# Axionis47/GAT-Recommendation

Hardware: AMD Instinct MI355X
Metric: training sessions/sec + Recall@10 parity, 82k-node graph, 1/2/4/8 MI355X (higher is better)
Workload: dtype fp32

## Files before the change

### gat-recommendation_amd/csrc/gtr_common.cuh

```cuda
#pragma once

#include <hip/hip_runtime.h>
#include <stdint.h>
#include <stdlib.h>

#include "../../include/gtr.h"

#define GTR_BLOCK 256
#define GTR_WAVES (GTR_BLOCK / 64)

typedef float f32x4 __attribute__((ext_vector_type(4)));

namespace gtr {

void set_error(const char* fmt, ...);

struct Buf {
  __amdgpu_buffer_rsrc_t r;
  __device__ __forceinline__ Buf(const void* p, uint64_t bytes)
      : r(__builtin_amdgcn_make_buffer_rsrc(const_cast<void*>(p), (short)0,
                                            (int)(uint32_t)(bytes < 0xFFFFFFFFull ? bytes : 0xFFFFFFFFull),
                                            0x00020000)) {}
  __device__ __forceinline__ float4 ld4(uint32_t off) const {
    return __builtin_bit_cast(float4, __builtin_amdgcn_raw_buffer_load_b128(r, (int)off, 0, 0));
// ... 158 lines not shown
  const int lane = threadIdx.x & 63;
  int lo = 0, hi = B;
  while (hi - lo > 64) {
    const int step = (hi - lo + 63) >> 6;
    const int idx = lo + lane * step;
    const int val = idx < hi ? a[idx] : 0x7FFFFFFF;
    const int c = __popcll(__ballot(val < v));
    const int nlo = c > 0 ? lo + (c - 1) * step + 1 : lo;
    const int nhi = min(hi, lo + c * step);
    lo = nlo;
    hi = nhi;
  }
  const int idx = lo + lane;
  const int val = idx < hi ? a[idx] : 0x7FFFFFFF;
  return lo + __popcll(__ballot(val < v));
}

__device__ __forceinline__ void group_rows(const int32_t* node_ptr, int B, int R, int g, int& r0, int& r1) {
  const int s0 = wave_lower_bound(node_ptr, B, g * R);
  const int s1 = wave_lower_bound(node_ptr, B, (g + 1) * R);
  r0 = node_ptr[s0];
  r1 = node_ptr[s1];
}

__device__ __forceinline__ int role_block(int M, int pack) {
  const int b = blockIdx.x;
  if (!pack) return b;
  if ((b & 7) == 0 && (b >> 3) < M) return b >> 3;
  return M + b - min(M, (b + 7) >> 3);
}

__device__ __forceinline__ bool arrive_last(uint32_t* cnt, uint32_t total, int* s_flag) {
  asm volatile("s_waitcnt vmcnt(0)" ::: "memory");
  __syncthreads();
  if (threadIdx.x == 0) {
    __builtin_amdgcn_fence(__ATOMIC_RELEASE, "agent");
    asm volatile("s_waitcnt vmcnt(0)" ::: "memory");
    uint32_t prev = __hip_atomic_fetch_add(cnt, 1u, __ATOMIC_RELAXED, __HIP_MEMORY_SCOPE_AGENT);
    *s_flag = (prev == total - 1) ? 1 : 0;
  }
  __syncthreads();
  if (*s_flag == 0) return false;
  if (threadIdx.x == 0) {
    __builtin_amdgcn_fence(__ATOMIC_ACQUIRE, "agent");
    asm volatile("s_waitcnt vmcnt(0)" ::: "memory");
  }
  __syncthreads();
  return true;
}

__device__ __forceinline__ void st_wt(float* p, float v) {
  __hip_atomic_store((__attribute__((address_space(1))) uint32_t*)(p), __float_as_uint(v),
                     __ATOMIC_RELAXED, __HIP_MEMORY_SCOPE_AGENT);
}

__device__ __forceinline__ bool arrive_last_wt(uint32_t* cnt, uint32_t total, int* s_flag) {
  asm volatile("s_waitcnt vmcnt(0)" ::: "memory");
  __syncthreads();
  if (threadIdx.x == 0) {
    uint32_t prev = __hip_atomic_fetch_add(cnt, 1u, __ATOMIC_RELAXED, __HIP_MEMORY_SCOPE_AGENT);
    *s_flag = (prev == total - 1) ? 1 : 0;
  }
  __syncthreads();
  if (*s_flag == 0) return false;
  if (threadIdx.x == 0) {
    __builtin_amdgcn_fence(__ATOMIC_ACQUIRE, "agent");
    asm volatile("s_waitcnt vmcnt(0)" ::: "memory");
  }
  __syncthreads();
  return true;
}

__device__ __forceinline__ void reset_counter(uint32_t* cnt) {
  __hip_atomic_store(cnt, 0u, __ATOMIC_RELAXED, __HIP_MEMORY_SCOPE_AGENT);
}

template <int BLK>
__device__ __forceinline__ void block_sum_rows(const float* p, int G, int W, size_t stride, float* out,
                                               float* scr, bool wt = false) {
  const int tid = threadIdx.x;
  if (W >= BLK) {
    for (int j = tid; j < W; j += BLK) {
      float acc = 0.0f;
#pragma unroll 32
      for (int q = 0; q < G; ++q) acc += p[(size_t)q * stride + j];
      if (wt) st_wt(out + j, acc); else out[j] = acc;
    }
    __syncthreads();
    return;
  }
  const int NSL = BLK / W;
  const int j = tid % W, sl = tid / W;
  if (sl < NSL) {
    float acc = 0.0f;
#pragma unroll 32
    for (int q = sl; q < G; q += NSL) acc += p[(size_t)q * stride + j];
    scr[sl * W + j] = acc;
  }
  __syncthreads();
  if (tid < W) {
    float t = 0.0f;
    for (int q = 0; q < NSL; ++q) t += scr[q * W + tid];
    if (wt) st_wt(out + tid, t); else out[tid] = t;
  }
  __syncthreads();
}
// ... 174 lines not shown
```

### gat-recommendation_amd/csrc/gtr_opt.hip

```cpp

#include <hipcub/hipcub.hpp>
#include <rocprim/device/device_radix_sort.hpp>

#include <cstdarg>
#include <cstdio>

#include "gtr_rows.cuh"
#include <string.h>

#include "gtr_wgrad.cuh"

namespace gtr {

static thread_local char g_err[512] = "";

void set_error(const char* fmt, ...) {
  va_list ap;
  va_start(ap, fmt);
  vsnprintf(g_err, sizeof(g_err), fmt, ap);
  va_end(ap);
}

}

// ... 521 lines not shown
      s_st.init(a.opt, t);
      s_t = (int32_t)t;
      s_ready = 1;
    }
    __syncthreads();
  }
  auto wait = [&]() {
    while (__hip_atomic_load(&s_ready, __ATOMIC_ACQUIRE, __HIP_MEMORY_SCOPE_WORKGROUP) == 0)
      __builtin_amdgcn_s_sleep(1);
  };
  const int blk = blockIdx.x;
  if (blk == 0 && tid == 0 && a.tl.rng_inc) *a.tl.rng_inc += 1;
  if (blk < a.nb_rows && a.windowed) {
    wait();
    const AdamStep st = s_st;
    window_rows<D>(blk, a.bt, a.T, a.tl, st, a.tl.lazy_consts ? a.tl.stamp : nullptr, s_t);
    return;
  }
  if (blk < a.nb_rows) {
    rows_body<D>(blk * GTR_BLOCK + tid, a.bt, a.T, a.tl.skeys, a.tl.svals, a.tl.dx0, a.tl.se, a.tl.coef_tgt,
                 a.tl.coef_neg, a.tl.table, a.tl.table_m, a.tl.table_v, nullptr, s_st,
                 a.tl.lazy_consts ? a.tl.stamp : nullptr, s_t, wait);
    return;
  }
  if (blk < a.nb_rows + a.nb_small) {
    const int sb = blk - a.nb_rows;
    small_body((int64_t)sb * GTR_BLOCK + tid, a.segs, a.nseg, a.bt.hdr, a.tl.flat, a.tl.flat_m, a.tl.flat_v, nullptr,
               s_st, wait);
    if (sb == 0 && a.tl.loss_part) {
      float acc = 0.0f;
      for (int q = tid; q < a.tl.loss_nparts; q += GTR_BLOCK)
        acc += a.tl.loss_part[(size_t)q * 2] + a.tl.loss_part[(size_t)q * 2 + 1];
      s_acc[tid] = acc;
      __syncthreads();
      if (tid == 0) {
        float t = 0.0f;
        for (int q = 0; q < GTR_BLOCK; ++q) t += s_acc[q];
        a.tl.loss_out[0] = t;
        if (a.tl.loss_acc) a.tl.loss_acc[0] += (double)t;
      }
    } else if (sb == 0 && a.tl.loss_acc && tid == 0) {
      a.tl.loss_acc[0] += (double)a.tl.loss_out[0];
    }
    return;
  }
  wait();
  const AdamStep st = s_st;
  sweep_body(blk - a.nb_rows - a.nb_small, a.nb_sweep, a.nvec, a.vpr_log2, a.tl.stamp, s_t,
             reinterpret_cast<float4*>(a.tl.table), reinterpret_cast<float4*>(a.tl.table_m),
             reinterpret_cast<float4*>(a.tl.table_v), st, a.vbegin);
}

#define GTR_TAILW_SEGS 16
#define GTR_WT_LIST 4352
struct TailWK {
  gtr_batch bt;
  gtr_tail tl;
  gtr_adam opt;
  int T, nb_rows, nb_wg, nb_small, njobs, D, nseg, P;
  int64_t stride;
  int small_total, pad0;
  uint32_t* cnt;
  gtr_segment segs[GTR_TAILW_SEGS];
  WJob jobs[GTR_MAX_WJOBS];
};

template <int D>
__global__ __launch_bounds__(GTR_BLOCK) void k_step_tail_wgrad(TailWK a) {
  __shared__ AdamStep s_st;
  __shared__ int32_t s_t;
  __shared__ float s_acc[GTR_BLOCK];
  __shared__ uint32_t s_list[GTR_WT_LIST];
  __shared__ int s_n;
  __shared__ int s_flag;
  const int tid = threadIdx.x;
  if (tid == 0) {
    const int64_t t = *a.opt.step_dev + a.opt.step_offset;
    s_st.init(a.opt, t);
    s_t = (int32_t)t;
    s_n = 0;
  }
  __syncthreads();
  const AdamStep st = s_st;
  int blk = blockIdx.x;
  if (blk == 0 && tid == 0 && a.tl.rng_inc) *a.tl.rng_inc += 1;
  if (blk < a.nb_wg) {
    int jid = 0;
    while (jid + 1 < a.njobs && blk >= a.jobs[jid + 1].blk0) ++jid;
    const WJob& J = a.jobs[jid];
    const int local = blk - J.blk0;
    const int tile = local / a.P, p = local - tile * a.P;
    const int N = a.bt.hdr[0];
    const int per = (N + a.P - 1) / a.P;
    const int t0 = p * per, t1 = min(N, t0 + per);
    const int64_t so = (int64_t)p * a.stride;
    auto rec = [&](uint32_t code) { s_list[atomicAdd(&s_n, 1)] = code; };
    auto emit = [&](int which, int64_t idx, float v) {
      if (which == 0) J.outW[so + idx] = v;
      else J.outB[so + idx] = v;
      rec(((uint32_t)which << 30) | (uint32_t)idx);
    };
    auto emit4 = [&](int64_t idx, float4 v) {
      *reinterpret_cast<float4*>(J.outW + so + idx) = v;
      rec((2u << 30) | (uint32_t)idx);
    };
    if (J.mfma == 1) wgrad_tile_mfma<false>(J, tile, t0, t1, emit, emit4);
    else if (J.mfma == 2) wgrad_tile_mfma<true>(J, tile, t0, t1, emit, emit4);
    else wgrad_tile(J, tile, t0, t1, a.D, emit);
    if (!arrive_last(a.cnt + J.tile0 + tile, (uint32_t)a.P, &s_flag)) return;
    const int n = s_n;
    float* P = a.tl.flat;
    float* M = a.tl.flat_m;
    float* V = a.tl.flat_v;
    for (int k = tid; k < n; k += GTR_BLOCK) {
      const uint32_t code = s_list[k];
      const uint32_t kind = code >> 30;
      const int64_t idx = code & 0x3FFFFFFFu;
      const float* src = kind == 1 ? J.outB : J.outW;
      const int64_t f0 = kind == 1 ? J.fB : J.fW;
      const int cnt = kind == 2 ? 4 : 1;
      for (int c = 0; c < cnt; ++c) {
        float g = 0.0f;
        for (int q = 0; q < a.P; ++q) g += src[(int64_t)q * a.stride + idx + c];
        const int64_t e = f0 + idx + c;
        float pv = P[e], mv = M[e], vv = V[e];
        st.apply(pv, mv, vv, g);
        P[e] = pv;
        M[e] = mv;
        V[e] = vv;
      }
    }
    if (tid == 0) reset_counter(a.cnt + J.tile0 + tile);
    return;
  }
  blk -= a.nb_wg;
  if (blk < a.nb_rows) {
    rows_body<D>(blk * GTR_BLOCK + tid, a.bt, a.T, a.tl.skeys, a.tl.svals, a.tl.dx0, a.tl.se, a.tl.coef_tgt,
                 a.tl.coef_neg, a.tl.table, a.tl.table_m, a.tl.table_v, nullptr, st,
                 a.tl.lazy_consts ? a.tl.stamp : nullptr, s_t);
    return;
  }
  blk -= a.nb_rows;
  if (blk < a.nb_small) {
    int64_t i = (int64_t)blk * GTR_BLOCK + tid;
    if (i < a.small_total) {
      int sg = 0;
      while (i >= a.segs[sg].len) { i -= a.segs[sg].len; ++sg; }
      const gtr_segment& S = a.segs[sg];
      float g = 0.0f;
      for (int q = 0; q < S.nparts; ++q) g += S.src[(int64_t)q * S.pstride + i];
      const int64_t e = S.begin + i;
      float pv = a.tl.flat[e], mv = a.tl.flat_m[e], vv = a.tl.flat_v[e];
      st.apply(pv, mv, vv, g);
      a.tl.flat[e] = pv;
      a.tl.flat_m[e] = mv;
      a.tl.flat_v[e] = vv;
    }
    if (blk == 0 && a.tl.loss_part) {
      float acc = 0.0f;
      for (int q = tid; q < a.tl.loss_nparts; q += GTR_BLOCK)
        acc += a.tl.loss_part[(size_t)q * 2] + a.tl.loss_part[(size_t)q * 2 + 1];
      s_acc[tid] = acc;
      __syncthreads();
      if (tid == 0) {
        float t = 0.0f;
        for (int q = 0; q < GTR_BLOCK; ++q) t += s_acc[q];
        a.tl.loss_out[0] = t;
        if (a.tl.loss_acc) a.tl.loss_acc[0] += (double)t;
      }
    } else if (blk == 0 && a.tl.loss_acc && tid == 0) {
      a.tl.loss_acc[0] += (double)a.tl.loss_out[0];
    }
  }
}

template <int D>
__global__ __launch_bounds__(GTR_BLOCK) void k_scatter_rows(gtr_batch bt, int mode, const float* src,
                                                            const float* coef_tgt, const float* coef_neg,
                                                            float* dense) {
  constexpr int VPL = D >= 64 ? D / 64 : 1;
  const int lane = threadIdx.x & 63, wave = threadIdx.x >> 6;
  const int r = blockIdx.x * GTR_WAVES + wave;
  const int d0 = lane * VPL;
  if (d0 >= D) return;
  const int N = bt.hdr[0], B = bt.hdr[1];
  int key;
  const float* s;
  float c;
  if (mode == 0) {
    if (r >= N) return;
    key = bt.node_item[r];
    s = src + (size_t)r * D;
    c = 1.0f;
  } else {
    if (r >= B * (1 + bt.n_neg)) return;
    if (r < B) {
      key = bt.target[r];
      s = src + (size_t)r * D;
      c = coef_tgt[r];
    } else {
      const int q = r - B;
      key = bt.negatives[q];
      s = src + (size_t)(q / bt.n_neg) * D;
      c = coef_neg[q];
    }
// ... 898 lines not shown
#define GTR_TAIL(DD) if (k.windowed) hipLaunchKernelGGL((k_step_tail<DD, false>), dim3(grid), dim3(GTR_BLOCK), 0, s, k); \
  else hipLaunchKernelGGL((k_step_tail<DD, true>), dim3(grid), dim3(GTR_TAIL_BLOCK), 0, s, k)
    case 32: GTR_TAIL(32); break;
    case 64: GTR_TAIL(64); break;
    case 128: GTR_TAIL(128); break;
    default: GTR_TAIL(256); break;
#undef GTR_TAIL
  }
  GTR_HIP_CHECK_LAUNCH();
  return GTR_OK;
}

int gtr_step_tail_wgrad(const gtr_config* cfg, const gtr_batch* bt, const gtr_layer* layers, const float* pe_tab,
                        float* const* layer_slab, float* pe_slab, int n_chunks, int64_t slab_stride,
                        const int64_t* layer_flat, const int64_t* pe_flat, int num_items, const gtr_tail* tail,
                        const gtr_segment* segs, int nseg, const gtr_adam* opt, uint32_t* tile_cnt, int tile_cnt_len,
                        gtr_stream_t stream) {
  if (!cfg || !bt || !layers || !layer_slab || !layer_flat || !tail || !opt || !opt->step_dev || num_items <= 0 ||
      nseg < 0 || nseg > GTR_TAILW_SEGS || (nseg > 0 && !segs) || !dim_ok(cfg->dim) || n_chunks <= 0 ||
      !tile_cnt || 3 * cfg->num_layers + 1 > GTR_MAX_WJOBS) {
    set_error("gtr_step_tail_wgrad: bad arguments");
    return GTR_E_ARG;
  }
  const gtr_tail& t = *tail;
  const int D = cfg->dim;
  const int m_cap = bt->n_cap + bt->b_cap * (1 + bt->n_neg);
  if (m_cap > GTR_BEGIN_MCAP) {
    set_error("gtr_step_tail_wgrad: batch too large (m_cap %d > %d): use gtr_wgrad + gtr_step_tail", m_cap,
              GTR_BEGIN_MCAP);
    return GTR_E_ARG;
  }
  if (!t.lazy_consts && t.sweep_from < num_items) {
    set_error("gtr_step_tail_wgrad: the untouched-row sweep must run in the chain (sweep_from == num_items)");
    return GTR_E_ARG;
  }
  if (!t.skeys || !t.svals || !t.dx0 || !t.se || !t.coef_tgt || !t.coef_neg || !t.table || !t.table_m ||
      !t.table_v || !t.stamp || !t.flat || !t.flat_m || !t.flat_v || (t.loss_part && (!t.loss_out || t.loss_nparts < 0))) {
    set_error("gtr_step_tail_wgrad: missing buffers");
    return GTR_E_ARG;
  }
  TailWK k{};
  k.bt = *bt;
  k.tl = t;
  k.opt = *opt;
  k.T = num_items;
  k.D = D;
  k.P = n_chunks;
  k.stride = slab_stride;
  k.cnt = tile_cnt;
  const char* wm = getenv("GTR_WGRAD");
  bool mfma = (bt->n_cap + n_chunks - 1) / n_chunks >= GTR_WGRAD_MFMA_ROWS;
  if (wm && !strcmp(wm, "mfma")) mfma = true;
  if (wm && !strcmp(wm, "valu")) mfma = false;
  if (slab_stride % 4) mfma = false;
  for (int l = 0; l < cfg->num_layers; ++l)
    if (reinterpret_cast<uintptr_t>(layer_slab[l]) % 16) mfma = false;
  int nj = 0, wblocks = 0;
  const int rc = build_wjobs(cfg, bt, layers, t.dx0, pe_tab, layer_slab, pe_slab, layer_flat, pe_flat, n_chunks, 0,
                             cfg->num_layers, k.jobs, nj, wblocks, mfma);
  if (rc) return rc;
  int tiles = 0;
  for (int i = 0; i < nj; ++i) {
    k.jobs[i].tile0 = tiles;
    tiles += k.jobs[i].nt;
    if (k.jobs[i].fW < 0 && k.jobs[i].fB < 0) { set_error("gtr_step_tail_wgrad: a job without flat offsets"); return GTR_E_ARG; }
  }
  if (tiles > tile_cnt_len) {
    set_error("gtr_step_tail_wgrad: %d tile counters needed, %d given", tiles, tile_cnt_len);
    return GTR_E_ARG;
  }
  k.njobs = nj;
  k.nb_wg = wblocks;
  k.nb_rows = (int)(((int64_t)m_cap * (D / 4) + GTR_BLOCK - 1) / GTR_BLOCK);
  int64_t tot = 0;
  for (int i = 0; i < nseg; ++i) {
    if (segs[i].live_groups) { set_error("gtr_step_tail_wgrad: folded (per row group) weight gradients"); return GTR_E_ARG; }
    k.segs[i] = segs[i];
    tot += segs[i].len;
  }
  k.nseg = nseg;
  k.small_total = (int)tot;
  k.nb_small = (int)((tot + GTR_BLOCK - 1) / GTR_BLOCK);
  if (k.nb_small == 0 && (t.loss_part || t.loss_acc)) k.nb_small = 1;
  const int grid = k.nb_wg + k.nb_rows + k.nb_small;
  hipStream_t s = (hipStream_t)stream;
  switch (D) {
    case 32: hipLaunchKernelGGL(k_step_tail_wgrad<32>, dim3(grid), dim3(GTR_BLOCK), 0, s, k); break;
    case 64: hipLaunchKernelGGL(k_step_tail_wgrad<64>, dim3(grid), dim3(GTR_BLOCK), 0, s, k); break;
    case 128: hipLaunchKernelGGL(k_step_tail_wgrad<128>, dim3(grid), dim3(GTR_BLOCK), 0, s, k); break;
    default: hipLaunchKernelGGL(k_step_tail_wgrad<256>, dim3(grid), dim3(GTR_BLOCK), 0, s, k); break;
  }
  GTR_HIP_CHECK_LAUNCH();
  return GTR_OK;
}

static bool dp_layout_ok(const gtr_dp_layout* l, int dim) {
  return l && l->world >= 1 && l->m_cap > 0 && l->flat_total >= 0 && l->loss_off >= l->flat_total &&
         l->keys_off > l->loss_off && l->rows_off >= l->keys_off + l->m_cap && (l->rows_off & 3) == 0 &&
         l->words >= l->rows_off + (int64_t)l->m_cap * dim && (l->words & 3) == 0;
}

int gtr_dp_pack(const gtr_batch* bt, int num_items, int dim, const gtr_tail* tail, const gtr_segment* segs, int nseg,
                const gtr_dp_layout* lay, float* pack, gtr_stream_t stream) {
  if (!bt || !tail || !pack || !dim_ok(dim) || !dp_layout_ok(lay, dim) || nseg < 0 || nseg > GTR_SMALL_MAX_SEG ||
      lay->m_cap != bt->n_cap + bt->b_cap * (1 + bt->n_neg) || !tail->skeys || !tail->svals || !tail->dx0 ||
      !tail->se || !tail->coef_tgt || !tail->coef_neg || (!tail->loss_part && !tail->loss_out)) {
    set_error("gtr_dp_pack: bad arguments");
    return GTR_E_ARG;
  }
  DpPackK k{};
  k.bt = *bt;
  k.tl = *tail;
  k.lay = *lay;
  k.pack = pack;
  k.T = num_items;
  hipStream_t s = (hipStream_t)stream;
  k.windowed = lay->m_cap > GTR_BEGIN_MCAP ? 1 : 0;
  if (k.windowed) {
    if (!tail->carry) { set_error("gtr_dp_pack: large batch (m_cap > %d) needs the carry scratch", GTR_BEGIN_MCAP); return GTR_E_ARG; }
    const int nwin = (lay->m_cap + TW - 1) / TW;
    k.nb_rows = nwin;
    if (nwin > 1) {
      switch (dim) {
        case 32: hipLaunchKernelGGL(k_tail_carry<32>, dim3(carry_blocks(lay->m_cap)), dim3(GTR_BLOCK), 0, s, *bt, num_items, *tail); break;
        case 64: hipLaunchKernelGGL(k_tail_carry<64>, dim3(carry_blocks(lay->m_cap)), dim3(GTR_BLOCK), 0, s, *bt, num_items, *tail); break;
        case 128: hipLaunchKernelGGL(k_tail_carry<128>, dim3(carry_blocks(lay->m_cap)), dim3(GTR_BLOCK), 0, s, *bt, num_items, *tail); break;
        default: hipLaunchKernelGGL(k_tail_carry<256>, dim3(carry_blocks(lay->m_cap)), dim3(GTR_BLOCK), 0, s, *bt, num_items, *tail); break;
      }
      GTR_HIP_CHECK_LAUNCH();
    }
  } else {
    k.nb_rows = (int)(((int64_t)lay->m_cap * (dim / 4) + GTR_BLOCK - 1) / GTR_BLOCK);
  }
  k.nb_small = (int)((lay->flat_total + GTR_BLOCK - 1) / GTR_BLOCK);
  if (k.nb_small == 0) k.nb_small = 1;
  k.nseg = nseg;
  for (int i = 0; i < nseg; ++i) k.segs[i] = segs[i];
  const int grid = k.nb_rows + k.nb_small;
  switch (dim) {
    case 32: hipLaunchKernelGGL(k_dp_pack<32>, dim3(grid), dim3(GTR_BLOCK), 0, s, k); break;
    case 64: hipLaunchKernelGGL(k_dp_pack<64>, dim3(grid), dim3(GTR_BLOCK), 0, s, k); break;
    case 128: hipLaunchKernelGGL(k_dp_pack<128>, dim3(grid), dim3(GTR_BLOCK), 0, s, k); break;
    default: hipLaunchKernelGGL(k_dp_pack<256>, dim3(grid), dim3(GTR_BLOCK), 0, s, k); break;
// ... 60 lines not shown
```

### gat-recommendation_amd/csrc/gtr_wgrad.cuh

```cuda
#pragma once

#include "gtr_common.cuh"

#include <type_traits>

namespace gtr {

enum { WJ_MM = 0, WJ_GATE = 1, WJ_COLSUM = 2 };

struct WJob {
  int type, M1, M2, lda, ldb, tn, nt, blk0;
  int mfma, wm, wn, fold_bias;
  const float* A;
  const float* B;
  const int32_t* bidx;
  const float* agg;
  const float* s;
  float* outW;
  float* outB;
  int64_t fW, fB;
  int tile0, pad_t;
};

#define GTR_MAX_WJOBS 16

#ifndef GTR_WGRAD_MFMA_ROWS
#define GTR_WGRAD_MFMA_ROWS 128
#endif

struct WgradK {
  const int32_t* hdr;
  int P, njobs, D, pad0;
  int64_t stride;
  WJob jobs[GTR_MAX_WJOBS];
};

template <class Emit>
__device__ __forceinline__ void wgrad_tile(const WJob& J, int tile, int t0, int t1, int D, Emit&& emit) {
  constexpr int TK = 32;
  __shared__ __attribute__((aligned(16))) float As[TK][64];
  __shared__ __attribute__((aligned(16))) float Bs[TK][64];
  const int tid = threadIdx.x;
  if (J.type == WJ_GATE || J.type == WJ_COLSUM) {
    constexpr int PH = GTR_BLOCK / 16;
    __shared__ float4 part[3][PH][16];
    const int c16 = tid & 15, ph = tid >> 4;
    const int col = tile * 64 + c16 * 4;
    const bool gate = J.type == WJ_GATE;
    const int ncol = gate ? D : J.M1;
    float4 g0 = make_float4(0.f, 0.f, 0.f, 0.f), g1 = g0, g2 = g0;
    if (col < ncol) {
      if (gate) {
        const float* ag = J.agg + col;
        const float* sk = J.s + col;
#pragma unroll 4
        for (int t = t0 + ph; t < t1; t += PH) {
          const float u = J.A[t];
          const float4 x = *reinterpret_cast<const float4*>(ag + (size_t)t * D);
          const float4 y = *reinterpret_cast<const float4*>(sk + (size_t)t * J.lda);
          g0.x += u * x.x; g0.y += u * x.y; g0.z += u * x.z; g0.w += u * x.w;
          g1.x += u * y.x; g1.y += u * y.y; g1.z += u * y.z; g1.w += u * y.w;
          g2.x += u * (x.x - y.x); g2.y += u * (x.y - y.y); g2.z += u * (x.z - y.z); g2.w += u * (x.w - y.w);
        }
      } else {
        const float* cp = J.A + col;
#pragma unroll 4
        for (int t = t0 + ph; t < t1; t += PH) {
          const float4 x = *reinterpret_cast<const float4*>(cp + (size_t)t * J.lda);
          g0.x += x.x; g0.y += x.y; g0.z += x.z; g0.w += x.w;
        }
      }
    }
    part[0][ph][c16] = g0;
    if (gate) {
      part[1][ph][c16] = g1;
      part[2][ph][c16] = g2;
    }
    __syncthreads();
    const int nseg = gate ? 3 : 1;
    if (tid < 64 * nseg) {
      const int sg = tid >> 6, cl = tid & 63, cc = cl >> 2, comp = cl & 3;
      const int j = tile * 64 + cl;
      float g = 0.0f;
#pragma unroll
      for (int q = 0; q < PH; ++q) {
        const float4 v = part[sg][q][cc];
        g += comp == 0 ? v.x : comp == 1 ? v.y : comp == 2 ? v.z : v.w;
      }
      if (j < ncol) {
        if (gate) emit(0, sg * D + j, g);
        else emit(1, j, g);
// ... 8 lines not shown
#pragma unroll
  for (int i = 0; i < 4; ++i)
#pragma unroll
    for (int k = 0; k < 4; ++k) acc[i][k] = 0.0f;
  constexpr int NQ = TK * 64 / GTR_BLOCK;
  float av[NQ], bv[NQ];
  auto load = [&](int tb) {
#pragma unroll
    for (int q = 0; q < NQ; ++q) {
      const int idx = tid + q * GTR_BLOCK;
      const int i = idx >> 6, c = idx & 63;
      const int t = tb + i;
      av[q] = 0.0f;
      bv[q] = 0.0f;
      if (t < t1) {
        if (m0 + c < J.M1) av[q] = J.A[(size_t)t * J.lda + m0 + c];
        const int col = n0 + c;
        if (col < J.M2) {
          const float* brow = J.bidx ? J.B + (size_t)J.bidx[t] * J.ldb : J.B + (size_t)t * J.ldb;
          bv[q] = brow[col];
        } else if (col == J.M2) {
          bv[q] = 1.0f;
        }
      }
    }
  };
  if (t0 < t1) load(t0);
  for (int tb = t0; tb < t1; tb += TK) {
#pragma unroll
    for (int q = 0; q < NQ; ++q) {
      const int idx = tid + q * GTR_BLOCK;
      As[idx >> 6][idx & 63] = av[q];
      Bs[idx >> 6][idx & 63] = bv[q];
    }
    __syncthreads();
    if (tb + TK < t1) load(tb + TK);
#pragma unroll 8
    for (int k = 0; k < TK; ++k) {
      const float4 a4 = *reinterpret_cast<const float4*>(&As[k][ty * 4]);
      const float4 b4 = *reinterpret_cast<const float4*>(&Bs[k][tx * 4]);
      const float ar[4] = {a4.x, a4.y, a4.z, a4.w};
      const float br[4] = {b4.x, b4.y, b4.z, b4.w};
#pragma unroll
      for (int i = 0; i < 4; ++i)
#pragma unroll
        for (int q = 0; q < 4; ++q) acc[i][q] += ar[i] * br[q];
    }
    __syncthreads();
  }
#pragma unroll
  for (int i = 0; i < 4; ++i) {
    const int m = m0 + ty * 4 + i;
    if (m >= J.M1) continue;
#pragma unroll
    for (int q = 0; q < 4; ++q) {
      const int nn = n0 + tx * 4 + q;
      if (nn < J.M2) emit(0, (int64_t)m * J.M2 + nn, acc[i][q]);
      else if (nn == J.M2) emit(1, m, acc[i][q]);
    }
  }
}

template <bool NARROW, class Emit, class Emit4>
__device__ __forceinline__ void wgrad_tile_mfma(const WJob& J, int tile, int t0, int t1, Emit&& emit, Emit4&& emit4) {
  constexpr int NT = NARROW ? 2 : 4;
  __shared__ f32x4 red[GTR_WAVES][4][64];
  const int tid = threadIdx.x, lane = tid & 63, wave = tid >> 6;
  const int nw = J.wm * J.wn, kw = GTR_WAVES / nw;
  const int wt = wave % nw, ks = wave / nw;
  const int tm = tile / J.tn, tq = tile - tm * J.tn;
  const int m0 = (tm * J.wm + wt % J.wm) * 64, n0 = (tq * J.wn + wt / J.wm) * 64;
  const int len = t1 - t0, per = (((len + kw - 1) / kw) + 3) & ~3;
  const int r0 = min(t1, t0 + ks * per), r1 = min(t1, r0 + per);
  const int kq = lane >> 4, c4 = (lane & 15) * 4, j16 = lane & 15;
  f32x4 acc[4][NT];
#pragma unroll
  for (int i = 0; i < 4; ++i)
#pragma unroll
    for (int q = 0; q < NT; ++q) acc[i][q] = f32x4{0.f, 0.f, 0.f, 0.f};
  const float* Ap = J.A + m0 + c4;
  const int rlast = max(0, r1 - 1);
  const int jb0 = min(j16, J.M2 - 1), jb1 = min(16 + j16, J.M2 - 1);
  const int32_t* ib = J.bidx ? J.bidx : reinterpret_cast<const int32_t*>(J.A);
  auto idx = [&](int t) -> int {
    const int tc = min(t, rlast);
    const int v = __builtin_nontemporal_load(ib + tc);
    return J.bidx ? v : tc;
  };
  auto ld = [&](int t, int bi, float4& a, float4& b) {
    const int tc = min(t, rlast);
    a = *reinterpret_cast<const float4*>(Ap + (size_t)tc * J.lda);
    if (NARROW) {
      const float* brow = J.B + (size_t)bi * J.ldb;
      b.x = brow[jb0];
      b.y = brow[jb1];
    } else {
      b = *reinterpret_cast<const float4*>(J.B + (size_t)tc * J.ldb + n0 + c4);
    }
  };
  auto fix = [&](int t, float4& a, float4& b) {
    if (t >= r1) {
      a = make_float4(0.f, 0.f, 0.f, 0.f);
      b = a;
    } else if (NARROW) {
      if (j16 >= J.M2) b.x = j16 == J.M2 ? 1.0f : 0.0f;
      if (16 + j16 >= J.M2) b.y = 16 + j16 == J.M2 ? 1.0f : 0.0f;
// ... 52 lines not shown
    stepk(std::integral_constant<int, 2>{}, t + 16);
  }
  if (colsum) {
    cs.x = bfly_add<32>(bfly_add<16>(cs.x)); cs.y = bfly_add<32>(bfly_add<16>(cs.y));
    cs.z = bfly_add<32>(bfly_add<16>(cs.z)); cs.w = bfly_add<32>(bfly_add<16>(cs.w));
  }
  for (int s = 1; s < kw; ++s) {
    if (colsum && ks == s) red[wt][0][lane] = f32x4{cs.x, cs.y, cs.z, cs.w};
    __syncthreads();
    if (colsum && ks == 0) {
      const f32x4 v = red[wt][0][lane];
      cs.x += v[0]; cs.y += v[1]; cs.z += v[2]; cs.w += v[3];
    }
    __syncthreads();
  }
  if (colsum && ks == 0 && kq == 0 && J.fold_bias) {
    emit(1, m0 + c4, cs.x);
    emit(1, m0 + c4 + 1, cs.y);
    emit(1, m0 + c4 + 2, cs.z);
    emit(1, m0 + c4 + 3, cs.w);
  }
  for (int mt = 0; mt < 4; ++mt) {
    for (int s = 1; s < kw; ++s) {
      if (ks == s) {
#pragma unroll
        for (int nt = 0; nt < NT; ++nt) red[wt][nt][lane] = acc[mt][nt];
      }
      __syncthreads();
      if (ks == 0) {
#pragma unroll
        for (int nt = 0; nt < NT; ++nt) acc[mt][nt] += red[wt][nt][lane];
      }
      __syncthreads();
    }
  }
  if (ks != 0) return;
#pragma unroll
  for (int mt = 0; mt < 4; ++mt)
#pragma unroll
    for (int r = 0; r < 4; ++r) {
      const int m = m0 + 16 * kq + 4 * r + mt;
      if (m >= J.M1) continue;
      if (NARROW) {
#pragma unroll
        for (int nt = 0; nt < NT; ++nt) {
          const int nn = 16 * nt + j16;
          if (nn < J.M2) emit(0, (int64_t)m * J.M2 + nn, acc[mt][nt][r]);
          else if (nn == J.M2) emit(1, m, acc[mt][nt][r]);
        }
      } else {
        emit4((int64_t)m * J.M2 + n0 + c4, make_float4(acc[mt][0][r], acc[mt][1][r], acc[mt][2][r], acc[mt][3][r]));
      }
    }
}

inline int build_wjobs(const gtr_config* cfg, const gtr_batch* bt, const gtr_layer* layers, const float* dx0,
                       const float* pe_tab, float* const* layer_slab, float* pe_slab, const int64_t* layer_flat,
                       const int64_t* pe_flat, int n_chunks, int l_begin, int l_end, WJob* jobs, int& nj,
                       int& blocks, bool mfma = false) {
  const int D = cfg->dim;
  nj = 0;
  blocks = 0;
  for (int l = l_begin; l < l_end; ++l) {
    const gtr_layer& L = layers[l];
    float* base = layer_slab ? layer_slab[l] : nullptr;
    const int64_t* fl = layer_flat ? layer_flat + 3 * l : nullptr;
    WJob& w = jobs[nj++];
    w = WJob{};
    w.type = WJ_MM; w.M1 = 4 * D; w.M2 = D; w.lda = 4 * D; w.ldb = D;
    w.tn = (D + 63) / 64; w.nt = ((4 * D + 63) / 64) * w.tn; w.blk0 = blocks;
    if (mfma && D % 64 == 0) {
      w.mfma = 1;
      w.wn = D / 64 >= 2 ? 2 : 1;
      w.wm = GTR_WAVES / w.wn < 4 * D / 64 ? GTR_WAVES / w.wn : 4 * D / 64;
      w.tn = D / (64 * w.wn);
      w.nt = (4 * D / (64 * w.wm)) * w.tn;
      w.fold_bias = 1;
    }
    w.A = L.dqkvs; w.B = L.xin; w.bidx = nullptr;
    w.outW = base; w.outB = base ? base + (size_t)4 * D * D : nullptr;
    w.fW = fl ? fl[0] : -1; w.fB = fl ? fl[1] : -1;
    blocks += w.nt * n_chunks;
    if (D % 64 == 0 && !w.mfma) {
      WJob& c = jobs[nj++];
      c = WJob{};
      c.type = WJ_COLSUM; c.M1 = 4 * D; c.lda = 4 * D; c.tn = 1; c.nt = (4 * D + 63) / 64;
      c.blk0 = blocks; c.A = L.dqkvs; c.outB = base ? base + (size_t)4 * D * D : nullptr;
      c.fW = -1; c.fB = fl ? fl[1] : -1;
      blocks += c.nt * n_chunks;
    }
    WJob& q = jobs[nj++];
    q = WJob{};
    q.type = WJ_GATE; q.M1 = 1; q.M2 = 3 * D; q.lda = 4 * D; q.tn = 1; q.nt = (D + 63) / 64;
    q.blk0 = blocks; q.A = L.du; q.agg = L.agg; q.s = L.qkvs + 3 * D;
    q.outW = base ? base + (size_t)4 * D * D + 4 * D : nullptr;
    q.fW = fl ? fl[2] : -1; q.fB = -1;
    blocks += q.nt * n_chunks;
  }
  if (cfg->pe_k > 0 && (pe_slab || pe_flat) && l_begin == 0) {
    if (!dx0 || (!pe_tab && !bt->node_pe)) { set_error("gtr_wgrad: PE gradient needs dx0 and PE rows"); return GTR_E_ARG; }
    const int K = cfg->pe_k;
    WJob& w = jobs[nj++];
    w = WJob{};
    w.type = WJ_MM; w.M1 = D; w.M2 = K; w.lda = D; w.ldb = K;
    w.tn = (K + 1 + 63) / 64; w.nt = ((D + 63) / 64) * w.tn; w.blk0 = blocks;
    w.A = dx0;
// ... 18 lines not shown
```

### gat-recommendation_amd/etpgt/train/fused.py

```python

from __future__ import annotations

import ctypes as C
import os

import torch

from etpgt.backend import _lib as L
from etpgt.backend.engine import Engine, readout_grid
from etpgt.data.batch import Caps, SessionBatch


class FusedTrainStep:
    def __init__(self, model, lr: float = 1e-3, betas=(0.9, 0.999), eps: float = 1e-8,
                 weight_decay: float = 1e-5, decoupled: bool = True, loss: str = "bpr",
                 temperature: float = 1.0, alpha: float = 0.7, caps: Caps | None = None,
                 use_graph: bool = True, data_parallel: bool | None = None, process_group=None,
                 lazy: bool = False, sync_bn: bool = False, lagged: bool = False, shard_table: bool = False):
        if loss not in ("bpr", "listwise", "dual", "sampled_softmax"):
            raise ValueError(f"Unknown loss type: {loss}")
        if getattr(model, "use_ffn", False):
            if os.environ.get("GTR_TAILW") == "1":
                raise NotImplementedError("the FFN variant (use_ffn=True) has no GTR_TAILW step")
            if sync_bn and not (model.embedding_dim in (64, 128) and getattr(model, "ffn_expansion", 4) == 4):
                raise NotImplementedError("SyncBN with the FFN variant covers dim 64 / 128 at ffn_expansion 4")
        self.model = model
        self.eng: Engine = model.hip_engine()
        self.dev = self.eng.device
        self.loss_kind = L.GTR_LOSS[loss]
        self.temperature = float(temperature)
        self.alpha = float(alpha)
        self.use_graph = use_graph
        from etpgt.train.distributed import world_info

        self.group = process_group
        self.rank, self.world = world_info(process_group)
        self.shard_table = bool(shard_table)
        if self.shard_table and (lazy or lagged):
            raise ValueError("the row-sharded table keeps its own lazy stamps (no lazy/lagged option)")
        self.data_parallel = (self.world > 1) if data_parallel is None else bool(data_parallel)
        self.data_parallel = self.data_parallel or self.shard_table

        self.sync_bn = bool(sync_bn)
        if self.sync_bn and not self.data_parallel:
            raise ValueError("sync_bn needs the data-parallel step")
        self.dp = None
        self.sync_alias = False
        self.graph_b = None
        self._coll_capture_refused = False
        eng = self.eng
        T, D = eng.T, eng.D
        self.adam = L.GtrAdam()
        self.adam.lr, self.adam.beta1, self.adam.beta2 = float(lr), float(betas[0]), float(betas[1])
        self.adam.eps, self.adam.weight_decay, self.adam.decoupled = float(eps), float(weight_decay), int(decoupled)
        self.step_dev = torch.zeros(1, dtype=torch.int64, device=self.dev)
        self.loss_acc = torch.zeros(1, dtype=torch.float64, device=self.dev)
        self.adam.step_dev = self.step_dev.data_ptr()
        self.adam.step_offset = 0
        tab_rows = 1 if self.shard_table else T
        self.m_tab = torch.zeros(tab_rows, D, dtype=torch.float32, device=self.dev)
        self.v_tab = torch.zeros(tab_rows, D, dtype=torch.float32, device=self.dev)
        self.m_flat = torch.zeros_like(eng.flat.flat)
        self.v_flat = torch.zeros_like(eng.flat.flat)
        self.stamp = torch.zeros(tab_rows, dtype=torch.int32, device=self.dev)
        self.lagged = bool(lagged) and not bool(lazy)
        self.lazy = bool(lazy) or self.lagged
# ... 143 lines not shown
        if self.begin_fused:
            wts[0] = 0.0
        self.early_union = (self.data_parallel and chain and not self.sync_bn and not self.lagged
                            and not self.shard_table and os.environ.get("GTR_DP_EARLY", "0") == "1")
        if self.early_union:
            wts = [0.0] * eng.L + wts[eng.L:]
        slots = len(wts)
        if chain and not self.shard_table and not self.split \
                and (not self.data_parallel or self.early_union or self.lagged) \
                and self.ws.g_cap <= 128 and slots <= L.SWEEP_SLOTS:
            sw = L.GtrSweep()
            sw.table = eng.model.item_embedding.weight.data_ptr()
            sw.m, sw.v, sw.stamp = self.m_tab.data_ptr(), self.v_tab.data_ptr(), self.stamp.data_ptr()
            sw.opt = self.adam
            tot, acc = sum(wts), 0.0
            if self.early_union:
                self.keys_all = torch.zeros(self.world, m_cap, dtype=torch.int32, device=self.dev)
            for i in range(L.SWEEP_SLOTS + 1):
                sw.bounds[i] = eng.T if i >= slots else int(eng.T * acc / tot)
                if i < slots:
                    acc += wts[i]
            sw.dim = eng.D
            sw.blocks = int(os.environ.get("GTR_SWEEP_BLOCKS", 0 if eng.D <= 64 else 128))
            sw.lag = 1 if self.lagged else 0
            sw.consts = self.lazy_consts.data_ptr() if self.lagged else None
            self.sweep = sw
            self.cfg.sweep = C.addressof(sw)
            t.sweep_from = eng.T
        t.lazy_consts = self.lazy_consts.data_ptr() if self.lazy else None
        nc = int(L.lib().gtr_tail_carry_floats(m_cap, eng.D))
        self.carry = torch.zeros(max(nc, 4), dtype=torch.float32, device=self.dev) if nc > 0 else None
        t.carry = self.carry.data_ptr() if self.carry is not None else None
        self.cfg.begin, self.cfg.ctr_add, t.rng_inc = None, 0, None
        if self.begin_fused:
            bg = L.GtrBegin()
            bg.skeys, bg.svals, bg.stamp = self.skeys.data_ptr(), self.svals.data_ptr(), self.stamp.data_ptr()
            bg.step_dev, bg.num_items = self.step_dev.data_ptr(), eng.T
            self.begin_st = bg
            self.cfg.begin = C.addressof(bg)
            self.cfg.ctr_add = 1
            t.rng_inc = eng.rng_ctr.data_ptr()
        self.tail = t
        if self.shard_table:
            from etpgt.train.sharded import ShardExchange

            self.dp = None
            self.shard = ShardExchange(self, self.shard_state)
        elif self.data_parallel:
            from etpgt.train.distributed import DpExchange

            self.dp = DpExchange(self, self.group)
        if self.sync_bn:
            self._sync_alloc()
        self.tail_wgrad = (self.dp is None and self.shard is None and m_cap <= 8192
                           and (self.lazy or t.sweep_from >= eng.T) and os.environ.get("GTR_TAILW", "0") == "1")
        if self.tail_wgrad:
            self.tile_cnt = torch.zeros(4096, dtype=torch.int32, device=self.dev)
            lay = eng.flat.layout
            gb = [i for i in range(self.nseg)
                  if any(self.segs[i].begin == lay.seg(f"{l}.{n}").begin for l in range(eng.L) for n in ("gamma", "beta"))]
            self.segs_gb = (L.GtrSegment * max(1, len(gb)))()
            for j, i in enumerate(gb):
                self.segs_gb[j] = self.segs[i]
            self.nseg_gb = len(gb)
            self.layer_flat = (C.c_int64 * (3 * eng.L))(*[lay.seg(f"{l}.{n}").begin for l in range(eng.L)
                                                          for n in ("w_all", "b_all", "w_beta")])
            self.pe_flat = (C.c_int64 * 2)(lay.seg("pe.w").begin, lay.seg("pe.b").begin) if eng.K > 0 else None
        self.graph = None
        self.graph_pe = None
        self.graph_b = None
        self.resident = None
        self.resident_graphs = None

    def workspace_ranges(self) -> list[tuple[str, int, int]]:
        out = []

        def add(name, t):
            if isinstance(t, torch.Tensor) and t.is_cuda and t.numel() > 0:
                out.append((name, t.data_ptr(), t.data_ptr() + t.numel() * t.element_size()))

        for name in ("keys", "vals", "skeys", "svals", "sort_tmp", "blob", "carry", "m_tab", "v_tab", "stamp",
                     "m_flat", "v_flat"):
            add(name, getattr(self, name, None))
        for name, t in vars(self.ws).items():
            add(f"ws.{name}", t)
        for l, lay in enumerate(getattr(self.ws, "layers", [])):
            for name, t in lay.items():
                add(f"ws.layers[{l}].{name}", t)
        return out

    def check_workspace_overlap(self) -> None:
        rs = sorted(self.workspace_ranges(), key=lambda r: r[1])
        for (n0, a0, b0), (n1, a1, b1) in zip(rs, rs[1:]):
            if a1 < b0 and not (a0 == a1 and b0 == b1):
                raise RuntimeError(f"workspace overlap: {n0} [{a0:#x}, {b0:#x}) and {n1} [{a1:#x}, {b1:#x})")

    def ensure_caps(self, batch: SessionBatch):
        N, B, E, n = batch.sizes()
        if self.data_parallel and self.world > 1:
            import torch.distributed as dist

            dev = self.dev if dist.get_backend(self.group) != "gloo" else "cpu"
            t = torch.tensor([N, B, E], dtype=torch.int64, device=dev)
            dist.all_reduce(t, op=dist.ReduceOp.MAX, group=self.group)
            N, B, E = (int(v) for v in t.tolist())
        if self.caps is None:
            self._bind(Caps.bucket(2 * N, B, 2 * E, n))
        elif not self.caps.fits(N, B, E, n):
# ... 653 lines not shown
```

Baseline: 431,600.

## Enable fused tail weight-grad step by default with structured tile finalize

Makes the fused tail weight-gradient kernel the default for single-device runs with small dimension and node cap, where before it needed an opt-in environment flag. The per-tile finalize no longer builds a shared-memory list of touched indices; it derives each tile's output region analytically and reduces the partials with batched, unrolled loads. Partial writes become write-through agent-scope stores, with vectorized buffer stores when aligned. An extra wavefront computes the Adam step constants while the other waves proceed, and they wait on it only just before applying the update. This removes shared-memory atomics, the serial step-constant load at kernel start and a separate launch path, at the cost of a larger block and added spin-wait synchronization.

```diff
diff --git a/gat-recommendation_amd/csrc/gtr_common.cuh b/gat-recommendation_amd/csrc/gtr_common.cuh
--- a/gat-recommendation_amd/csrc/gtr_common.cuh
+++ b/gat-recommendation_amd/csrc/gtr_common.cuh
@@ -234,6 +234,12 @@
 __device__ __forceinline__ void st_wt(float* p, float v) {
   __hip_atomic_store((__attribute__((address_space(1))) uint32_t*)(p), __float_as_uint(v),
                      __ATOMIC_RELAXED, __HIP_MEMORY_SCOPE_AGENT);
+}
+
+template <class Rsrc>
+__device__ __forceinline__ void st_wt4(Rsrc rsrc, int off, float4 v) {
+  const f32x4 x = {v.x, v.y, v.z, v.w};
+  __builtin_amdgcn_raw_buffer_store_b128(x, rsrc, off, 0, 16);
 }
 
 __device__ __forceinline__ bool arrive_last_wt(uint32_t* cnt, uint32_t total, int* s_flag) {
diff --git a/gat-recommendation_amd/csrc/gtr_opt.hip b/gat-recommendation_amd/csrc/gtr_opt.hip
--- a/gat-recommendation_amd/csrc/gtr_opt.hip
+++ b/gat-recommendation_amd/csrc/gtr_opt.hip
@@ -597,36 +597,101 @@
 }
 
 #define GTR_TAILW_SEGS 16
-#define GTR_WT_LIST 4352
 struct TailWK {
   gtr_batch bt;
   gtr_tail tl;
   gtr_adam opt;
   int T, nb_rows, nb_wg, nb_small, njobs, D, nseg, P;
   int64_t stride;
-  int small_total, pad0;
+  int small_total, vec;
   uint32_t* cnt;
   gtr_segment segs[GTR_TAILW_SEGS];
   WJob jobs[GTR_MAX_WJOBS];
 };
 
+template <int EB, class Wait>
+__device__ __forceinline__ void tile_finalize(const WOut& R, int P, int64_t stride, float* fp, float* fm, float* fv,
+                                              const AdamStep& s_st, Wait wait) {
+  const int tid = threadIdx.x;
+  const int dq = GTR_BLOCK / R.wc, dr = GTR_BLOCK - dq * R.wc;
+  for (int base = 0; base < R.count; base += EB * GTR_BLOCK) {
+    int off[EB];
+    uint32_t isb = 0, on = 0;
+    int i = (base + tid) / R.wc, c = base + tid - i * R.wc;
+#pragma unroll
+    for (int k = 0; k < EB; ++k) {
+      const bool in = base + tid + k * GTR_BLOCK < R.count;
+      const int ic = in ? i : 0, cc = in ? c : 0;
+      const bool bias = cc >= R.nw;
+      off[k] = bias ? R.m0 + ic : (R.m0 + ic) * R.ld + R.n0 + cc;
+      on |= (uint32_t)in << k;
+      isb |= (uint32_t)bias << k;
+      i += dq;
+      c += dr;
+      if (c >= R.wc) { c -= R.wc; ++i; }
+    }
+    float pv[EB], mv[EB], vv[EB], g[EB];
+#pragma unroll
+    for (int k = 0; k < EB; ++k) {
+      const int64_t fe = ((isb >> k) & 1 ? R.fb : R.fw) + off[k];
+      pv[k] = fp[fe];
+      mv[k] = fm[fe];
+      vv[k] = fv[fe];
+      g[k] = 0.0f;
+    }
+    for (int q0 = 0; q0 < P; q0 += 8) {
+      float x[8][EB];
+#pragma unroll
+      for (int u = 0; u < 8; ++u) {
+        const int64_t qo = (int64_t)min(q0 + u, P - 1) * stride;
+#pragma unroll
+        for (int k = 0; k < EB; ++k) x[u][k] = ((isb >> k) & 1 ? R.b : R.w)[qo + off[k]];
+      }
+#pragma unroll
+      for (int u = 0; u < 8; ++u) {
+        if (q0 + u >= P) break;
+#pragma unroll
+        for (int k = 0; k < EB; ++k) g[k] += x[u][k];
+      }
+    }
+    wait();
+    const AdamStep st = s_st;
+#pragma unroll
+    for (int k = 0; k < EB; ++k) {
+      st.apply(pv[k], mv[k], vv[k], g[k]);
+      if ((on >> k) & 1) {
+        const int64_t fe = ((isb >> k) & 1 ? R.fb : R.fw) + off[k];
+        fp[fe] = pv[k];
+        fm[fe] = mv[k];
+        fv[fe] = vv[k];
+      }
+    }
+  }
+}
+
 template <int D>
-__global__ __launch_bounds__(GTR_BLOCK) void k_step_tail_wgrad(TailWK a) {
+__global__ __launch_bounds__(GTR_TAIL_BLOCK) void k_step_tail_wgrad(TailWK a) {
   __shared__ AdamStep s_st;
   __shared__ int32_t s_t;
+  __shared__ int s_ready;
   __shared__ float s_acc[GTR_BLOCK];
-  __shared__ uint32_t s_list[GTR_WT_LIST];
-  __shared__ int s_n;
   __shared__ int s_flag;
   const int tid = threadIdx.x;
-  if (tid == 0) {
-    const int64_t t = *a.opt.step_dev + a.opt.step_offset;
-    s_st.init(a.opt, t);
-    s_t = (int32_t)t;
-    s_n = 0;
-  }
+  if (tid == 0) s_ready = 0;
   __syncthreads();
-  const AdamStep st = s_st;
+  if (tid >= GTR_BLOCK) {
+    if (tid == GTR_BLOCK) {
+      const int64_t t = *a.opt.step_dev + a.opt.step_offset;
+      s_st.init(a.opt, t);
+      s_t = (int32_t)t;
+      __hip_atomic_store(&s_ready, 1, __ATOMIC_RELEASE, __HIP_MEMORY_SCOPE_WORKGROUP);
+    }
+    return;
+  }
+  auto wait = [&]() {
+    while (__hip_atomic_load(&s_ready, __ATOMIC_ACQUIRE, __HIP_MEMORY_SCOPE_WORKGROUP) == 0)
+      __builtin_amdgcn_s_sleep(1);
+  };
   int blk = blockIdx.x;
   if (blk == 0 && tid == 0 && a.tl.rng_inc) *a.tl.rng_inc += 1;
   if (blk < a.nb_wg) {
@@ -639,50 +704,29 @@
     const int per = (N + a.P - 1) / a.P;
     const int t0 = p * per, t1 = min(N, t0 + per);
     const int64_t so = (int64_t)p * a.stride;
-    auto rec = [&](uint32_t code) { s_list[atomicAdd(&s_n, 1)] = code; };
-    auto emit = [&](int which, int64_t idx, float v) {
-      if (which == 0) J.outW[so + idx] = v;
-      else J.outB[so + idx] = v;
-      rec(((uint32_t)which << 30) | (uint32_t)idx);
-    };
-    auto emit4 = [&](int64_t idx, float4 v) {
-      *reinterpret_cast<float4*>(J.outW + so + idx) = v;
-      rec((2u << 30) | (uint32_t)idx);
+    auto emit = [&](int which, int64_t idx, float v) { st_wt((which == 0 ? J.outW : J.outB) + so + idx, v); };
+    const auto rs = __builtin_amdgcn_make_buffer_rsrc(J.outW + so, 0, J.M1 * J.M2 * 4, 0x00020000);
+    auto emit4 = [&](int64_t idx, float4 v) -> bool {
+      if (!a.vec || (idx & 3) || (reinterpret_cast<uintptr_t>(J.outW) & 15)) return false;
+      st_wt4(rs, (int)idx * 4, v);
+      return true;
     };
     if (J.mfma == 1) wgrad_tile_mfma<false>(J, tile, t0, t1, emit, emit4);
     else if (J.mfma == 2) wgrad_tile_mfma<true>(J, tile, t0, t1, emit, emit4);
-    else wgrad_tile(J, tile, t0, t1, a.D, emit);
-    if (!arrive_last(a.cnt + J.tile0 + tile, (uint32_t)a.P, &s_flag)) return;
-    const int n = s_n;
-    float* P = a.tl.flat;
-    float* M = a.tl.flat_m;
-    float* V = a.tl.flat_v;
-    for (int k = tid; k < n; k += GTR_BLOCK) {
-      const uint32_t code = s_list[k];
-      const uint32_t kind = code >> 30;
-      const int64_t idx = code & 0x3FFFFFFFu;
-      const float* src = kind == 1 ? J.outB : J.outW;
-      const int64_t f0 = kind == 1 ? J.fB : J.fW;
-      const int cnt = kind == 2 ? 4 : 1;
-      for (int c = 0; c < cnt; ++c) {
-        float g = 0.0f;
-        for (int q = 0; q < a.P; ++q) g += src[(int64_t)q * a.stride + idx + c];
-        const int64_t e = f0 + idx + c;
-        float pv = P[e], mv = M[e], vv = V[e];
-        st.apply(pv, mv, vv, g);
-        P[e] = pv;
-        M[e] = mv;
-        V[e] = vv;
-      }
-    }
+    else wgrad_tile(J, tile, t0, t1, a.D, emit, emit4);
+    if (!arrive_last_wt(a.cnt + J.tile0 + tile, (uint32_t)a.P, &s_flag)) return;
+    const WOut R = wgrad_outputs(J, tile, a.D);
+    if (R.count <= GTR_BLOCK) tile_finalize<1>(R, a.P, a.stride, a.tl.flat, a.tl.flat_m, a.tl.flat_v, s_st, wait);
+    else if (R.count <= 8 * GTR_BLOCK) tile_finalize<8>(R, a.P, a.stride, a.tl.flat, a.tl.flat_m, a.tl.flat_v, s_st, wait);
+    else tile_finalize<16>(R, a.P, a.stride, a.tl.flat, a.tl.flat_m, a.tl.flat_v, s_st, wait);
     if (tid == 0) reset_counter(a.cnt + J.tile0 + tile);
     return;
   }
   blk -= a.nb_wg;
   if (blk < a.nb_rows) {
     rows_body<D>(blk * GTR_BLOCK + tid, a.bt, a.T, a.tl.skeys, a.tl.svals, a.tl.dx0, a.tl.se, a.tl.coef_tgt,
-                 a.tl.coef_neg, a.tl.table, a.tl.table_m, a.tl.table_v, nullptr, st,
-                 a.tl.lazy_consts ? a.tl.stamp : nullptr, s_t);
+                 a.tl.coef_neg, a.tl.table, a.tl.table_m, a.tl.table_v, nullptr, s_st,
+                 a.tl.lazy_consts ? a.tl.stamp : nullptr, s_t, wait);
     return;
   }
   blk -= a.nb_rows;
@@ -692,10 +736,20 @@
       int sg = 0;
       while (i >= a.segs[sg].len) { i -= a.segs[sg].len; ++sg; }
       const gtr_segment& S = a.segs[sg];
-      float g = 0.0f;
-      for (int q = 0; q < S.nparts; ++q) g += S.src[(int64_t)q * S.pstride + i];
       const int64_t e = S.begin + i;
       float pv = a.tl.flat[e], mv = a.tl.flat_m[e], vv = a.tl.flat_v[e];
+      float g = 0.0f;
+      const int np = S.nparts;
+      for (int q0 = 0; q0 < np; q0 += 8) {
+        float x[8];
+#pragma unroll
+        for (int u = 0; u < 8; ++u) x[u] = S.src[(int64_t)min(q0 + u, np - 1) * S.pstride + i];
+#pragma unroll
+        for (int u = 0; u < 8; ++u)
+          if (q0 + u < np) g += x[u];
+      }
+      wait();
+      const AdamStep st = s_st;
       st.apply(pv, mv, vv, g);
       a.tl.flat[e] = pv;
       a.tl.flat_m[e] = mv;
@@ -1700,6 +1754,9 @@
   bool mfma = (bt->n_cap + n_chunks - 1) / n_chunks >= GTR_WGRAD_MFMA_ROWS;
   if (wm && !strcmp(wm, "mfma")) mfma = true;
   if (wm && !strcmp(wm, "valu")) mfma = false;
+  k.vec = slab_stride % 4 == 0;
+  for (int l = 0; l < cfg->num_layers; ++l)
+    if (reinterpret_cast<uintptr_t>(layer_slab[l]) % 16) k.vec = 0;
   if (slab_stride % 4) mfma = false;
   for (int l = 0; l < cfg->num_layers; ++l)
     if (reinterpret_cast<uintptr_t>(layer_slab[l]) % 16) mfma = false;
@@ -1733,10 +1790,10 @@
   const int grid = k.nb_wg + k.nb_rows + k.nb_small;
   hipStream_t s = (hipStream_t)stream;
   switch (D) {
-    case 32: hipLaunchKernelGGL(k_step_tail_wgrad<32>, dim3(grid), dim3(GTR_BLOCK), 0, s, k); break;
-    case 64: hipLaunchKernelGGL(k_step_tail_wgrad<64>, dim3(grid), dim3(GTR_BLOCK), 0, s, k); break;
-    case 128: hipLaunchKernelGGL(k_step_tail_wgrad<128>, dim3(grid), dim3(GTR_BLOCK), 0, s, k); break;
-    default: hipLaunchKernelGGL(k_step_tail_wgrad<256>, dim3(grid), dim3(GTR_BLOCK), 0, s, k); break;
+    case 32: hipLaunchKernelGGL(k_step_tail_wgrad<32>, dim3(grid), dim3(GTR_TAIL_BLOCK), 0, s, k); break;
+    case 64: hipLaunchKernelGGL(k_step_tail_wgrad<64>, dim3(grid), dim3(GTR_TAIL_BLOCK), 0, s, k); break;
+    case 128: hipLaunchKernelGGL(k_step_tail_wgrad<128>, dim3(grid), dim3(GTR_TAIL_BLOCK), 0, s, k); break;
+    default: hipLaunchKernelGGL(k_step_tail_wgrad<256>, dim3(grid), dim3(GTR_TAIL_BLOCK), 0, s, k); break;
   }
   GTR_HIP_CHECK_LAUNCH();
   return GTR_OK;
diff --git a/gat-recommendation_amd/csrc/gtr_wgrad.cuh b/gat-recommendation_amd/csrc/gtr_wgrad.cuh
--- a/gat-recommendation_amd/csrc/gtr_wgrad.cuh
+++ b/gat-recommendation_amd/csrc/gtr_wgrad.cuh
@@ -35,8 +35,13 @@
   WJob jobs[GTR_MAX_WJOBS];
 };
 
-template <class Emit>
-__device__ __forceinline__ void wgrad_tile(const WJob& J, int tile, int t0, int t1, int D, Emit&& emit) {
+struct NoEmit4 {
+  __device__ __forceinline__ bool operator()(int64_t, float4) const { return false; }
+};
+
+template <class Emit, class Emit4 = NoEmit4>
+__device__ __forceinline__ void wgrad_tile(const WJob& J, int tile, int t0, int t1, int D, Emit&& emit,
+                                           Emit4&& emit4 = Emit4{}) {
   constexpr int TK = 32;
   __shared__ __attribute__((aligned(16))) float As[TK][64];
   __shared__ __attribute__((aligned(16))) float Bs[TK][64];
@@ -151,6 +156,9 @@
   for (int i = 0; i < 4; ++i) {
     const int m = m0 + ty * 4 + i;
     if (m >= J.M1) continue;
+    if (n0 + tx * 4 + 3 < J.M2 &&
+        emit4((int64_t)m * J.M2 + n0 + tx * 4, make_float4(acc[i][0], acc[i][1], acc[i][2], acc[i][3])))
+      continue;
 #pragma unroll
     for (int q = 0; q < 4; ++q) {
       const int nn = n0 + tx * 4 + q;
@@ -309,6 +317,44 @@
         emit4((int64_t)m * J.M2 + n0 + c4, make_float4(acc[mt][0][r], acc[mt][1][r], acc[mt][2][r], acc[mt][3][r]));
       }
     }
+}
+
+struct WOut {
+  const float* w;
+  const float* b;
+  int64_t fw, fb;
+  int ld, m0, n0, nw, wc, count;
+};
+
+__device__ __forceinline__ WOut wgrad_outputs(const WJob& J, int tile, int D) {
+  WOut R;
+  R.w = J.outW; R.b = J.outB; R.fw = J.fW; R.fb = J.fB;
+  int rows;
+  if (J.type == WJ_GATE) {
+    R.ld = D; R.m0 = 0; R.n0 = tile * 64; R.nw = min(64, D - R.n0); R.wc = R.nw;
+    rows = 3;
+  } else if (J.type == WJ_COLSUM) {
+    R.w = J.outB; R.fw = J.fB;
+    R.ld = 0; R.m0 = 0; R.n0 = tile * 64; R.nw = min(64, J.M1 - R.n0); R.wc = R.nw;
+    rows = 1;
+  } else {
+    const int tm = tile / J.tn, tq = tile - tm * J.tn;
+    int hasb;
+    R.ld = J.M2;
+    if (J.mfma == 1) {
+      R.m0 = tm * J.wm * 64; rows = J.wm * 64;
+      R.n0 = tq * J.wn * 64; R.nw = J.wn * 64;
+      hasb = J.fold_bias && tq == 0;
+    } else {
+      R.m0 = tm * 64; rows = 64;
+      R.n0 = tq * 64; R.nw = max(0, min(64, J.M2 - R.n0));
+      hasb = J.M2 >= R.n0 && J.M2 < R.n0 + 64;
+    }
+    rows = min(rows, J.M1 - R.m0);
+    R.wc = R.nw + hasb;
+  }
+  R.count = max(0, rows) * max(0, R.wc);
+  return R;
 }
 
 inline int build_wjobs(const gtr_config* cfg, const gtr_batch* bt, const gtr_layer* layers, const float* dx0,
diff --git a/gat-recommendation_amd/etpgt/train/fused.py b/gat-recommendation_amd/etpgt/train/fused.py
--- a/gat-recommendation_amd/etpgt/train/fused.py
+++ b/gat-recommendation_amd/etpgt/train/fused.py
@@ -12,6 +12,9 @@
 
 
 class FusedTrainStep:
+    TAILW_MAX_DIM = 64
+    TAILW_MAX_N_CAP = 512
+
     def __init__(self, model, lr: float = 1e-3, betas=(0.9, 0.999), eps: float = 1e-8,
                  weight_decay: float = 1e-5, decoupled: bool = True, loss: str = "bpr",
                  temperature: float = 1.0, alpha: float = 0.7, caps: Caps | None = None,
@@ -261,8 +264,15 @@
             self.dp = DpExchange(self, self.group)
         if self.sync_bn:
             self._sync_alloc()
-        self.tail_wgrad = (self.dp is None and self.shard is None and m_cap <= 8192
-                           and (self.lazy or t.sweep_from >= eng.T) and os.environ.get("GTR_TAILW", "0") == "1")
+        can_tailw = (self.dp is None and self.shard is None and m_cap <= 8192
+                     and (self.lazy or t.sweep_from >= eng.T))
+        tailw = os.environ.get("GTR_TAILW")
+        if tailw in ("0", "1"):
+            self.tail_wgrad = can_tailw and tailw == "1"
+        else:
+            self.tail_wgrad = (can_tailw and not getattr(self.model, "use_ffn", False) and not self.split
+                               and os.environ.get("GTR_WFOLD", "0") != "1"
+                               and eng.D <= self.TAILW_MAX_DIM and caps.n_cap <= self.TAILW_MAX_N_CAP)
         if self.tail_wgrad:
             self.tile_cnt = torch.zeros(4096, dtype=torch.int32, device=self.dev)
             lay = eng.flat.layout
```

New measurement: 434,400, median of 6. No clear change (+0.6%).
